# vrgamegirl19/comfyui-vrgamedevgirl

Measured on AMD Instinct MI355X. Metric: Mpixels/s (grain+LUT+colormatch+sharpen) at 4K, higher is better.
Workload: dtype f32

## Files before the change

comfyui-vrgamedevgirl_amd/csrc/vrg_chain.hip:

```cpp
#include "vrg_common.hpp"
#include <type_traits>
#include "vrg_chain_stages.hpp"

namespace vrg {

constexpr int STATS_BPF_MAX = 128;
constexpr int STATS_PX_PER_BLOCK = 16384;

__host__ __device__ inline int stats_blocks_per_frame(int64_t pixels) {
    int64_t b = (pixels + STATS_PX_PER_BLOCK - 1) / STATS_PX_PER_BLOCK;
    return (int)(b < 1 ? 1 : (b > STATS_BPF_MAX ? STATS_BPF_MAX : b));
}

template <int STAGES, class IO>
__global__ __launch_bounds__(256) void k_chain_pointwise(const typename IO::elem* __restrict__ in, typename IO::elem* __restrict__ out,
                                                          int32_t ppf, ChainK D) {
    VRG_CM_MATH(PT, (STAGES & VRG_STAGE_COLORMATCH) != 0, (STAGES & VRG_STAGE_FASTMATH) != 0, D.dm);
    const int32_t p = blockIdx.x * 256 + threadIdx.x;
    if (p >= ppf) return;
    const int64_t f = blockIdx.y;
    const px3 v = IO::load_stream(in + f * ppf + p);
    const float x[3] = {v.r, v.g, v.b};
    float o[3];
    chain_pre<STAGES>(D, frame_ctx<STAGES>(D, f), p, x, o, PT);
// ... 8 lines not shown
    px3 v[4];
#pragma unroll
    for (int j = 0; j < 4; ++j) {
        const int32_t p = p0 + 256 * j;
        v[j] = load_px_stream(fin + (p < ppf ? p : 0));
    }
    VRG_CM_MATH(PT, true, (STAGES & VRG_STAGE_FASTMATH) != 0, D.dm);
    typedef unsigned u3 __attribute__((ext_vector_type(3)));
    const __amdgpu_buffer_rsrc_t rs = __builtin_amdgcn_make_buffer_rsrc(reinterpret_cast<void*>(out + f * ppf), 0, ppf * 12, 0x00020000);
    const FrameCtx FC = frame_ctx<STAGES>(D, f);
#pragma unroll
    for (int j = 0; j < 4; ++j) {
        const int32_t p = p0 + 256 * j;
        const bool valid = p < ppf;
        const float x[3] = {v[j].r, v[j].g, v[j].b};
        float o[3];
        chain_pre<STAGES>(D, FC, valid ? p : 0, x, o, PT);
        __builtin_amdgcn_raw_buffer_store_b96(u3{__float_as_uint(o[0]), __float_as_uint(o[1]), __float_as_uint(o[2])}, rs,
                                              (int)(valid ? (uint32_t)p * 12u : 0x80000000u), 0, 0);
    }
}

#define VRG_TILE_H 32
constexpr int TILE_H = VRG_TILE_H, TILE_W = 64;
constexpr int TILE_ROWS = TILE_H / 4;
constexpr int HALO_H = TILE_H + 2, HALO_W = TILE_W + 2;
constexpr int LDS_PITCH = HALO_W + 1;

template <int STAGES, class IO>
__global__ __launch_bounds__(256) void k_chain_tile(const typename IO::elem* __restrict__ in, typename IO::elem* __restrict__ out,
                                                     int32_t H, int32_t W, int32_t tiles_x, int32_t tiles_per_frame, uint32_t total_work,
                                                     ChainK D) {
    __shared__ float tile[3][HALO_H][LDS_PITCH];
    VRG_CM_MATH(PT, (STAGES & VRG_STAGE_COLORMATCH) != 0, (STAGES & VRG_STAGE_FASTMATH) != 0, D.dm);
    const uint32_t per_xcd = (total_work + 7u) / 8u;
    const uint32_t work = (blockIdx.x & 7u) * per_xcd + (blockIdx.x >> 3);
    if ((blockIdx.x >> 3) >= per_xcd || work >= total_work) return;
    const uint32_t tile_id = work % (uint32_t)tiles_per_frame;
    const int32_t ty0 = (int32_t)(tile_id / (uint32_t)tiles_x) * TILE_H;
    const int32_t tx0 = (int32_t)(tile_id % (uint32_t)tiles_x) * TILE_W;
    const int64_t f = work / (uint32_t)tiles_per_frame;
    const int32_t ppf = H * W;
    const typename IO::elem* fin = in + f * ppf;
    const bool zero = D.zero_border != 0;
    const FrameCtx FC = frame_ctx<STAGES>(D, f);

#define VRG_TILE_PRELOAD 1
    constexpr int N_IT = (HALO_H * HALO_W + 255) / 256;
    if (VRG_TILE_PRELOAD && !(STAGES & VRG_STAGE_COLORMATCH) && !((STAGES & VRG_STAGE_GRAIN) && !(STAGES & VRG_STAGE_LUT))) {
        px3 v[N_IT];
        int32_t pp[N_IT];
#pragma unroll
        for (int k = 0; k < N_IT; ++k) {
            int i = (int)threadIdx.x + 256 * k;
            i = i < HALO_H * HALO_W ? i : 0;
            const int hy = i / HALO_W, hx = i - hy * HALO_W;
            int y = ty0 + hy - 1, x = tx0 + hx - 1;
            y = y < 0 ? 0 : (y > H - 1 ? H - 1 : y);
            x = x < 0 ? 0 : (x > W - 1 ? W - 1 : x);
            pp[k] = y * W + x;
            v[k] = IO::load(fin + pp[k]);
        }
#pragma unroll
        for (int k = 0; k < N_IT; ++k) {
            const int i = (int)threadIdx.x + 256 * k;
            if (i < HALO_H * HALO_W) {
                const int hy = i / HALO_W, hx = i - hy * HALO_W;
// ... 448 lines not shown
```

comfyui-vrgamedevgirl_amd/csrc/vrg_common.hpp:

```cpp
#pragma once

#if !defined(VRG_LAB_VARIANT_SOURCE) && (defined(VRG_APPLY_EARLY_LOAD) || defined(VRG_APPLY_ROWS) || defined(VRG_FLAT_ROWS) || defined(VRG_GRAIN_NT) || \
    defined(VRG_PRODUCE_MAX_WAVES_LABONLY) || defined(VRG_PRODUCE_WAVES) || defined(VRG_PRODUCE_WAVES_LABONLY) || defined(VRG_PR_PIPE) || \
    defined(VRG_PR_SUBS) || defined(VRG_SG_PIPE) || defined(VRG_TILE_H) || defined(VRG_TILE_PRELOAD) || \
    defined(VRG_TS_LANES) || defined(VRG_TS_LANES_DEPTH) || defined(VRG_TS_LANES_MAX_FRAMES) || defined(VRG_TS_LANES_MEAN_DEPTH) || \
    defined(VRG_TS_MARKSTEIN) || defined(VRG_TS_ROWS_DEPTH) || defined(VRG_TS_ROWS_MAX_FRAMES) || defined(VRG_TS_SPLIT_DEPTH) || \
    defined(VRG_TS_SPLIT_MAX_FRAMES) || defined(VRG_TS_WHOLE_DEPTH) || defined(VRG_ZIV_REL) || defined(VRG_MARCH_FAST) || \
    defined(VRG_MARCH_MIN_WAVES) || defined(VRG_MARCH_FINITE) || defined(VRG_MARCH_ABLATE) || defined(VRG_MARCH_QUAD) || \
    defined(VRG_MARCH_ENDIO) || defined(VRG_MARCH_ROTATE) || defined(VRG_MARCH_TAPS_UNFOLD) || defined(VRG_MARCH_FAST_FLAT) || \
    defined(VRG_MARCH_EDGE_SHARED) || defined(VRG_MARCH_FAST_LDS) || defined(VRG_NO_POINTWISE4) || defined(VRG_NO_APPLY_MARCH) || \
    defined(VRG_NO_FLAT_STENCIL) || defined(VRG_APPLY_FORCE_GENERAL) || defined(VRG_ABLATE_GATHER) || defined(VRG_NO_DIVT_FASTPATH))
#error "comfyui-vrgamedevgirl_amd: tuning / ablation macros are not build options of the product sources (see the note above this line)"
#endif
#include <stdint.h>

#include "../../include/vrgdg_hip.h"
#include "../../include/vrgdg_hip_debug.h"
#include "vrg_pixel_math.hpp"

namespace vrg {

VRG_HD bool span_fits(int64_t offset, int64_t need, int64_t size) { return offset >= 0 && offset <= size && need <= size - offset; }

constexpr int64_t LAUNCH_RECORDS = 32768;
// ... 72 lines not shown
    int64_t chunk0;
    int64_t frame_elems;
    int32_t chunk_frames;
    uint32_t G;
};

VRG_HD uint64_t chunk_seed(const NoiseK& n, int64_t chunk_rel) { return n.seed0 + (uint64_t)(n.chunk0 + chunk_rel) * n.seed_stride; }
VRG_HD uint64_t chunk_offset(const NoiseK& n, int64_t chunk_rel) { return n.off0 + (uint64_t)(n.chunk0 + chunk_rel) * n.off_stride; }

struct CmK {
    const float* img_ms;
    const float* ref_ms;
    int32_t ref_frames;
    float K, T;
};

struct ChainK {
    int32_t stages;
    float I, S, T;
    NoiseK noise;
    LutParams lut;
    CmK cm;
    DevMath dm;
    int32_t stencil_op, zero_border;
    float strength;
};

constexpr int VRG_STAGE_FASTMATH = 32;

inline DevMath host_dev_math() { return DevMath{(float)2.4, (float)(1.0 / 2.4), (float)(1.0 / 3.0), nullptr}; }

template <bool FAST> struct CmMathSel { typedef DevMath type; };
template <> struct CmMathSel<true> { typedef PowTables type; };
__device__ __forceinline__ PowTables cm_make_math(const float* lds, const DevMath&, const PowTables*) { return PowTables{lds, lds + 512}; }
__device__ __forceinline__ DevMath cm_make_math(const float* lds, const DevMath& dm, const DevMath*) {
    DevMath m = dm;
    m.logt = lds;
    return m;
}

inline NoiseK make_noise(const vrg_noise_desc* d, int64_t frame_elems) {
    NoiseK n;
    n.seed0 = d->seed0; n.seed_stride = d->seed_stride; n.off0 = d->offset0; n.off_stride = d->offset_stride;
    n.chunk0 = d->chunk0; n.frame_elems = frame_elems; n.chunk_frames = d->chunk_frames; n.G = d->grid_threads;
    return n;
}

inline LutParams make_lut(const float* cells, int n, const float dmin[3], const float dmax[3], int blend_mode,
                          float blend, float one_minus_blend) {
    LutParams P;
    P.cells = cells; P.n = n; P.top = (float)(n - 1);
    P.unit_domain = 1;
    for (int c = 0; c < 3; ++c) {
        P.dmin[c] = dmin[c];
        const float span = dmax[c] - dmin[c];
        P.span[c] = span < 1e-6f ? 1e-6f : span;
        if (!(P.dmin[c] == 0.0f && P.span[c] == 1.0f)) P.unit_domain = 0;
    }
    P.blend_mode = blend_mode; P.blend = blend; P.one_minus_blend = one_minus_blend;
    return P;
}

#define VRG_CM_MATH(PT, NEED, FAST, DM)                                                                       \
    __shared__ __attribute__((aligned(16))) float vrg_pow_lds_[(NEED) ? ((FAST) ? ::vrg::POW_TABLE_WORDS : ::vrg::ZIV_TABLE_WORDS) : 4]; \
    if (NEED) {                                                                                                \
        if (FAST) ::vrg::pow_tables_fill(vrg_pow_lds_, (int)threadIdx.x, (int)blockDim.x);                    \
        else ::vrg::ziv_table_fill(vrg_pow_lds_, (int)threadIdx.x, (int)blockDim.x);                          \
        __syncthreads();                                                                                       \
    }                                                                                                          \
    typedef typename ::vrg::CmMathSel<(FAST)>::type PT##_t;                                                    \
    const PT##_t PT = ::vrg::cm_make_math(vrg_pow_lds_, (DM), (const PT##_t*)nullptr)

#define VRG_CHECK_LAUNCH()                                   \
    do {                                                     \
        hipError_t e_ = hipGetLastError();                   \
        if (e_ != hipSuccess) return VRG_ERR_LAUNCH;         \
    } while (0)

template <class T, int N>
__device__ __forceinline__ void block_sum_4waves(T (&acc)[N], T (&part)[4][N]) {
#pragma unroll
    for (int i = 0; i < N; ++i) {
#pragma unroll
        for (int off = 32; off >= 1; off >>= 1) acc[i] += __shfl_xor(acc[i], off, 64);
    }
    const int wave = threadIdx.x >> 6, lane = threadIdx.x & 63;
    if (lane == 0) {
#pragma unroll
        for (int i = 0; i < N; ++i) part[wave][i] = acc[i];
    }
    __syncthreads();
}

}
#endif
```

comfyui-vrgamedevgirl_amd/csrc/vrg_pixel_math.hpp:

```cpp
#pragma once
#include <stdint.h>

#if defined(__HIPCC__) || defined(__HIP__)
#include <hip/hip_runtime.h>
#define VRG_HD __host__ __device__ __forceinline__
#define VRG_D __device__ __forceinline__
#else
#define VRG_HD inline
#define VRG_D inline
#endif

#ifndef VRG_HW_LOG2
#define VRG_HW_LOG2(x) __builtin_amdgcn_logf(x)
#define VRG_HW_SIN_REV(x) __builtin_amdgcn_sinf(x)
#define VRG_HW_COS_REV(x) __builtin_amdgcn_cosf(x)
#define VRG_HW_EXP2(x) __builtin_amdgcn_exp2f(x)
#define VRG_HW_RCP(x) __builtin_amdgcn_rcpf(x)
#endif

namespace vrg {

VRG_HD float f32_from_bits(uint32_t b) {
    union { uint32_t u; float f; } c;
    c.u = b;
// ... 428 lines not shown
VRG_HD void pow_tables_fill(float* dst, int first, int stride) {
    for (int i = first; i < POW_TABLE_WORDS; i += stride)
        dst[i] = f32_from_bits(i < 512 ? VRG_POW_LOGT[i >> 2][i & 3] : VRG_POW_EXPT[(i - 512) >> 1][(i - 512) & 1]);
}

VRG_HD float pow_pos(float x, float y, const PowTables& T) {
    union { float f; uint32_t u; } cv;
    cv.f = x;
    const uint32_t b = cv.u;
    const float e = (float)((int)(b >> 23) - 127);
    const uint32_t i = (b >> 16) & 0x7fu;
    const float m = f32_from_bits((b & 0x007fffffu) | 0x3f800000u);
    const float invc = T.logt[4 * i], lhi = T.logt[4 * i + 1], llo = T.logt[4 * i + 2];
    const float r = __builtin_fmaf(m, invc, -1.0f);
    float p = __builtin_fmaf(r, f32_from_bits(VRG_POW_A[2]), f32_from_bits(VRG_POW_A[1]));
    p = __builtin_fmaf(r, p, f32_from_bits(VRG_POW_A[0]));
    const float L_hi = e + lhi;
    const float L_lo = __builtin_fmaf(r, p, llo);
    const float E_hi = y * L_hi;
    const float E_lo = __builtin_fmaf(y, L_lo, __builtin_fmaf(y, L_hi, -E_hi));
    const float nf = __builtin_rintf(E_hi * 64.0f);
    const float f = __builtin_fmaf(nf, -0.015625f, E_hi) + E_lo;
    const int n = (int)nf;
    float q = __builtin_fmaf(f, f32_from_bits(VRG_POW_B[3]), f32_from_bits(VRG_POW_B[2]));
    q = __builtin_fmaf(f, q, f32_from_bits(VRG_POW_B[1]));
    q = __builtin_fmaf(f, q, f32_from_bits(VRG_POW_B[0]));
    q = f * q;
    const float thi = T.expt[2 * (n & 63)], tlo = T.expt[2 * (n & 63) + 1];
    const float v = thi + __builtin_fmaf(thi, q, tlo);
    const float res = __builtin_ldexpf(v, n >> 6);
    return (x != x) ? x : res;
}

struct DevMath {
    float e24, e1_24, e1_3;
    const float* logt;
};

#if defined(__HIP_DEVICE_COMPILE__)
extern "C" __device__ float __ocml_pow_f32(float, float);
#define VRG_LIB_POWF(x, y) __ocml_pow_f32((x), (y))
#define VRG_HW_FREXP_MANT(x) __builtin_amdgcn_frexp_mantf(x)
#define VRG_HW_FREXP_EXP(x) __builtin_amdgcn_frexp_expf(x)
#else
#define VRG_LIB_POWF(x, y) __builtin_powf((x), (y))
#define VRG_HW_FREXP_MANT(x) __builtin_frexpf((x), &vrg_frexp_dummy_)
#define VRG_HW_FREXP_EXP(x) ::vrg::host_frexp_exp(x)
static int vrg_frexp_dummy_;
VRG_HD int host_frexp_exp(float x) { int e; (void)__builtin_frexpf(x, &e); return e; }
#endif

constexpr int DEV_POW_ANY = 0, DEV_POW_OVF = 1, DEV_POW_UNIT = 2;

VRG_HD float dev_exp_core(float x) {
    const float c = f32_from_bits(0x3fb8aa3bu);
    const float ph = x * c;
    const float f0 = __builtin_fmaf(x, c, -ph);
    const float pl = __builtin_fmaf(x, f32_from_bits(0x32a5705fu), f0);
    const float e = __builtin_rintf(ph);
    const float a = (ph - e) + pl;
    return __builtin_ldexpf(VRG_HW_EXP2(a), (int)e);
}

VRG_HD float dev_exp_core_normal(float x) {
    const float c = f32_from_bits(0x3fb8aa3bu);
    const float ph = x * c;
    const float f0 = __builtin_fmaf(x, c, -ph);
    const float pl = __builtin_fmaf(x, f32_from_bits(0x32a5705fu), f0);
    const float magic = f32_from_bits(0x4b400000u);
// ... 119 lines not shown
    float ln_hi, ln_lo;
    dev_epln<GUARD>(x, ln_hi, ln_lo);
    const float p17 = y * ln_hi;
    const float p24 = __builtin_fmaf(y, ln_hi, -p17);
    const float p44 = __builtin_fmaf(y, ln_lo, p24);
    const float p50 = p17 + p44;
    const float p51 = p50 - p17;
    const float p52 = p44 - p51;
    const float inf = __builtin_inff();
    const float ovf = f32_from_bits(0x42b17218u);
    float ph = p50, pl = p52;
    if (GUARD == DEV_POW_ANY) {
        ph = (__builtin_fabsf(p17) == inf) ? p17 : p50;
        pl = (__builtin_fabsf(ph) == inf) ? 0.0f : p52;
    }
    float h5 = ph, l7 = pl;
    if (GUARD != DEV_POW_UNIT) {
        const float c4 = (ph == ovf) ? f32_from_bits(0x37000000u) : 0.0f;
        h5 = ph - c4;
        l7 = pl + c4;
    }
    float e8 = dev_exp_core(h5);
    if (GUARD == DEV_POW_ANY) e8 = (h5 < f32_from_bits(0xc2ce8ed0u)) ? 0.0f : e8;
    if (GUARD != DEV_POW_UNIT) e8 = (h5 > ovf) ? inf : e8;
    const float r9 = __builtin_fmaf(e8, l7, e8);
    const float r = (GUARD != DEV_POW_UNIT && __builtin_fabsf(e8) == inf) ? e8 : r9;
    if (GUARD == DEV_POW_ANY) return (x == inf) ? (y > 0.0f ? inf : 0.0f) : r;
    return (x < inf) ? r : ((x == inf) ? (y > 0.0f ? inf : 0.0f) : x);
}
VRG_HD float dev_pow(float x, float y) { return dev_pow_t<DEV_POW_ANY>(x, y); }

#include "vrg_ziv_log_table.inc"

constexpr int ZIV_TABLE_WORDS = 128 * 4;

VRG_HD void ziv_table_fill(float* dst, int first, int stride) {
    for (int i = first; i < ZIV_TABLE_WORDS; i += stride) dst[i] = f32_from_bits(VRG_ZIV_LOGT[i >> 2][i & 3]);
}

VRG_HD void ziv_log(float x, const float* T, float& Lh, float& Ll, float& Eh_out, float& A_out) {
    const int32_t d = (int32_t)(f32_bits(x) - 0x3f2aaaabu);
    const uint32_t e23 = (uint32_t)d & 0xff800000u;
    const float ef23 = (float)(int32_t)e23;
    const float m = f32_from_bits(f32_bits(x) - e23);
    const float* t = T + (((uint32_t)d >> 16) & 0x7fu) * 4;
    const float c = t[0], th = t[1], tl = t[2];
    A_out = t[3];
    const float r = __builtin_fmaf(m, c, -1.0f);
    const float Eh = ef23 * f32_from_bits(0x33b17200u);
    const float h = r * r;
    const float l = __builtin_fmaf(r, r, -h);
    float P = __builtin_fmaf(r, (float)(-1.0 / 6.0), 0.2f);
    P = __builtin_fmaf(r, P, -0.25f);
    P = __builtin_fmaf(r, P, (float)(1.0 / 3.0));
    const float tail = __builtin_fmaf(-0.5f, l, (h * r) * P);
    const float s1 = Eh + th;
    const float s2 = __builtin_fmaf(-0.5f, h, r);
    const float e2 = __builtin_fmaf(-0.5f, h, r - s2);
    const float s3 = s1 + s2;
    const float e3 = s2 - (s3 - s1);
    float low = __builtin_fmaf(ef23, f32_from_bits(0x2a3fbe8eu), tl);
    low = low + e3;
    low = low + e2;
    low = low + tail;
    Lh = s3;
    Ll = low;
    Eh_out = Eh;
}

#define VRG_ZIV_REL 1
#define VRG_ZIV_REL_BITS 0x2e06f428u
VRG_HD float ziv_delta(float Lh, float Eh, float A_over_C) {
#if VRG_ZIV_REL
    const float rel = __builtin_fmaf(__builtin_fabsf(Eh), 64.0f, __builtin_fabsf(Lh));
#if defined(__HIP_DEVICE_COMPILE__)
    return __builtin_amdgcn_fmed3f(rel, A_over_C, 0.0f);
#else
    return __builtin_fminf(rel, A_over_C);
#endif
#else
    (void)Lh; (void)Eh;
    return A_over_C;
#endif
}

template <bool IN_DOMAIN = false>
VRG_HD bool ziv_try(float x, float y, const float* T, uint32_t lo_bits, uint32_t hi_bits, float& out) {
    float Lh, Ll, Eh, A;
    ziv_log(x, T, Lh, Ll, Eh, A);
    const float p17 = y * Lh;
    const float p24 = __builtin_fmaf(y, Lh, -p17);
    const float p44 = __builtin_fmaf(y, Ll, p24);
    const float yc = y * f32_from_bits(VRG_ZIV_REL_BITS);
    const float dl = ziv_delta(Lh, Eh, A);
    const float up = __builtin_fmaf(yc, dl, p44), dn = __builtin_fmaf(-yc, dl, p44);
    const float php = p17 + up;
    const float phm = p17 + dn;
    const float t = php - p17;
    const float e8 = dev_exp_core_normal(php);
    const float rp = __builtin_fmaf(e8, up - t, e8);
    const float rm = __builtin_fmaf(e8, dn - t, e8);
    out = rp;
    if (IN_DOMAIN) return (php == phm) & (rp == rm);
    return ((f32_bits(x) - lo_bits) <= (hi_bits - lo_bits)) & (php == phm) & (rp == rm);
}

template <int GUARD>
VRG_HD float dev_pow_ziv(float x, float y, const float* T, uint32_t lo_bits, uint32_t hi_bits) {
#if defined(__HIP_DEVICE_COMPILE__)
    if (T) {
        float r;
        if (ziv_try(x, y, T, lo_bits, hi_bits, r)) return r;
#if defined(VRG_LAB_VARIANT_SOURCE) && defined(LAB_ZIV_NO_FALLBACK)
        return r;
#endif
    }
#else
    (void)T; (void)lo_bits; (void)hi_bits;
#endif
    return dev_pow_t<GUARD>(x, y);
}

template <int GUARD, bool IN_DOMAIN = false>
VRG_HD void dev_pow_ziv3(const float x[3], float y, const float* T, uint32_t lo_bits, uint32_t hi_bits, float o[3]) {
#if defined(__HIP_DEVICE_COMPILE__)
    if (T) {
        float r0, r1, r2;
        const bool dom = IN_DOMAIN || __builtin_fmaxf(__builtin_fmaxf(x[0], x[1]), x[2]) <= f32_from_bits(hi_bits);
        const bool s0 = ziv_try<true>(x[0], y, T, lo_bits, hi_bits, r0) & dom;
        const bool s1 = ziv_try<true>(x[1], y, T, lo_bits, hi_bits, r1) & dom;
        const bool s2 = ziv_try<true>(x[2], y, T, lo_bits, hi_bits, r2) & dom;
        o[0] = r0; o[1] = r1; o[2] = r2;
#if defined(VRG_LAB_VARIANT_SOURCE) && defined(LAB_ZIV_NO_FALLBACK)
        if (s0 | s1 | s2 | true) return;
#endif
        if (!s0) o[0] = dev_pow_t<GUARD>(x[0], y);
        if (!s1) o[1] = dev_pow_t<GUARD>(x[1], y);
        if (!s2) o[2] = dev_pow_t<GUARD>(x[2], y);
        return;
    }
#else
    (void)T; (void)lo_bits; (void)hi_bits;
#endif
#pragma unroll
    for (int c = 0; c < 3; ++c) o[c] = dev_pow_t<GUARD>(x[c], y);
}

VRG_HD float cm_div_scalar(float x, float c, float rc, float, const PowTables&) { return div_const(x, c, rc); }
VRG_HD float cm_div_scalar(float x, float, float, float rc_dev, const DevMath&) { return x * rc_dev; }
#define VRG_CM_DIVS(x, c, M) ::vrg::cm_div_scalar((x), (float)(c), 1.0f / (float)(c), (float)(1.0 / (double)(c)), (M))
VRG_HD float cm_div_tensor(float x, float c, float rc, const PowTables&) { return div_const(x, c, rc); }
VRG_HD float cm_div_tensor(float x, float c, float rc, const DevMath&) {
#if defined(__HIP_DEVICE_COMPILE__)
    const bool proven = ((__builtin_fabsf(x) - 1e-30f) <= (1e30f - 1e-30f)) | (x == 0.0f);
    if (__builtin_amdgcn_ballot_w64(!proven) == 0) return div_const(x, c, rc);
#else
    (void)rc;
#endif
    return x / c;
// ... 281 lines not shown
```

comfyui-vrgamedevgirl_amd/csrc/vrg_probe.hip:

```cpp
#include "vrg_common.hpp"
#include "vrg_lanes.hpp"
#include "vrg_tstats_config.hpp"

namespace vrg {

__global__ __launch_bounds__(256) void k_selftest_divconst(unsigned long long* counts, uint32_t first) {
    const uint32_t bits = first + blockIdx.x * 256u + threadIdx.x;
    const float x = f32_from_bits(bits);
    if (x != x) return;
    const float a = __builtin_fabsf(x);
    const bool mid = a >= 1e-30f && a <= 1e30f;
    float got[9], want[9];
    got[0] = VRG_DIVC(x, 1.055f);   want[0] = x / 1.055f;
    got[1] = VRG_DIVC(x, 12.92f);   want[1] = x / 12.92f;
    got[2] = VRG_DIVC(x, 0.95047f); want[2] = x / 0.95047f;
    got[3] = VRG_DIVC(x, 1.08883f); want[3] = x / 1.08883f;
    got[4] = VRG_DIVC(x, 116.0f);   want[4] = x / 116.0f;
    got[5] = VRG_DIVC(x, 500.0f);   want[5] = x / 500.0f;
    got[6] = VRG_DIVC(x, 200.0f);   want[6] = x / 200.0f;
    got[7] = VRG_DIVC(x, 7.787f);   want[7] = x / 7.787f;
    got[8] = div9(x);               want[8] = x / 9.0f;
#pragma unroll
    for (int w = 0; w < 9; ++w) {
        const bool same = (got[w] == want[w]) || (got[w] != got[w] && want[w] != want[w]);
// ... 180 lines not shown
            acc[j] = 0.0f;
        }
        for (int pass = 0; pass < 3; ++pass) {
            __syncthreads();
            const f32x4* src = reinterpret_cast<const f32x4*>(cells + (size_t)pass * total);
            f32x4* dst = reinterpret_cast<f32x4*>(dbg_nodes);
            for (int i = threadIdx.x; i < (total + 3) / 4; i += 1024) dst[i] = src[i];
            __syncthreads();
            const float* T = dbg_nodes;
#pragma unroll
            for (int j = 0; j < PX; ++j) {
                const int bs = base[j];
                acc[j] += (T[bs] + T[bs + 1]) + (T[bs + n] + T[bs + n + 1]);
                acc[j] += (T[bs + n * n] + T[bs + n * n + 1]) + (T[bs + n * n + n] + T[bs + n * n + n + 1]);
            }
        }
#pragma unroll
        for (int j = 0; j < PX; ++j) {
            const int64_t p = b0 + j * 1024 + threadIdx.x;
            if (p < pixels) out[p] = acc[j];
        }
    }
}

__global__ __launch_bounds__(256) void k_dbg_cm_math(const float* __restrict__ in, float* __restrict__ out, int64_t n, int op, float y,
                                                      DevMath dm) {
    VRG_CM_MATH(PT, true, true, dm);
    __shared__ __attribute__((aligned(16))) float zivt[ZIV_TABLE_WORDS];
    ziv_table_fill(zivt, (int)threadIdx.x, 256);
    __syncthreads();
    dm.logt = zivt;
    const int64_t i = (int64_t)blockIdx.x * 256 + threadIdx.x;
    if (i >= n) return;
    if (op == 20) {
        const float lab = in[3 * i], mu = in[3 * i + 1], sd = in[3 * i + 2];
        const float ms[6] = {mu, sd, mu, sd, mu, sd};
        const SigmaRecip R = sigma_recip(ms);
        const float d = lab - mu;
        out[3 * i] = div_sigma_unscaled(d, sd, R.y1[0]);
        out[3 * i + 1] = d / sd;
        out[3 * i + 2] = (R.usable && (__builtin_fabsf(d) + __builtin_fabsf(d)) + __builtin_fabsf(d) < 0x1p40f) ? 1.0f : 0.0f;
    } else if (op >= 16) {
        float a, b;
        float eh, aj;
        if (op <= 17) dev_epln<DEV_POW_UNIT>(in[i], a, b); else ziv_log(in[i], zivt, a, b, eh, aj);
        out[i] = (op & 1) ? b : a;
    } else if (op >= 12) {
        const float x = in[i];
        if (op == 12) out[i] = dev_pow_ziv<DEV_POW_OVF>(x, y, zivt, 0x3d800000u, 0x40000000u);
        else if (op == 13) out[i] = dev_pow_ziv<DEV_POW_UNIT>(x, y, zivt, 0x3b4d2e1cu, 0x40800000u);
        else if (op == 14) out[i] = dev_pow_ziv<DEV_POW_UNIT>(x, y, zivt, 0x3c1118c2u, 0x40800000u);
        else {
            float r;
            out[i] = ziv_try(x, y, zivt, 0x00800000u, 0x7f7fffffu, r) ? 0.0f : 1.0f;
        }
    } else if (op >= 9) {
        out[i] = op == 9 ? dev_pow_t<DEV_POW_ANY>(in[i], y) : (op == 10 ? dev_pow_t<DEV_POW_OVF>(in[i], y) : dev_pow_t<DEV_POW_UNIT>(in[i], y));
    } else if (op <= 4) {
        const float x = in[i];
        float r;
        if (op == 0) r = VRG_LIB_POWF(x, y);
        else if (op == 1) r = x * (float)(1.0 / (double)y);
        else if (op == 2) r = x / y;
        else if (op == 3) r = pow_pos(x, y, PT);
        else r = cbrt_pow(x);
        out[i] = r;
    } else {
        const float x[3] = {in[3 * i], in[3 * i + 1], in[3 * i + 2]};
        float o[3];
        if (op == 5) rgb_to_lab(x, o, dm);
        else if (op == 6) lab_to_rgb(x, o, dm);
        else if (op == 7) rgb_to_lab(x, o, PT);
        else lab_to_rgb(x, o, PT);
        out[3 * i] = o[0]; out[3 * i + 1] = o[1]; out[3 * i + 2] = o[2];
    }
}

}

namespace vrg {

template <int MODE>
__global__ __launch_bounds__(256) void k_dbg_copy(const f32x4* __restrict__ in, f32x4* __restrict__ out, int64_t n4) {
    if (MODE == 0 || MODE == 1) {
        const int64_t i = (int64_t)blockIdx.x * 256 + threadIdx.x;
        if (i >= n4) return;
        if (MODE == 0) out[i] = in[i];
// ... 308 lines not shown
    hipStream_t st = (hipStream_t)stream;
#define VRG_VALU_CASE(M) case M: hipLaunchKernelGGL(vrg::k_dbg_valu_rate<M>, dim3(blocks), dim3(256), 0, st, out, iters); break;
    switch (mode) {
        VRG_VALU_CASE(0) VRG_VALU_CASE(1) VRG_VALU_CASE(2) VRG_VALU_CASE(3) VRG_VALU_CASE(4) VRG_VALU_CASE(5) VRG_VALU_CASE(6) VRG_VALU_CASE(7) VRG_VALU_CASE(8) VRG_VALU_CASE(9) VRG_VALU_CASE(10) VRG_VALU_CASE(11) VRG_VALU_CASE(12) VRG_VALU_CASE(13) VRG_VALU_CASE(14) VRG_VALU_CASE(15) VRG_VALU_CASE(16) VRG_VALU_CASE(17) VRG_VALU_CASE(18) VRG_VALU_CASE(19) VRG_VALU_CASE(20) VRG_VALU_CASE(21) VRG_VALU_CASE(30) VRG_VALU_CASE(31) VRG_VALU_CASE(32) VRG_VALU_CASE(33) VRG_VALU_CASE(34) VRG_VALU_CASE(35) VRG_VALU_CASE(36) VRG_VALU_CASE(37) VRG_VALU_CASE(38) VRG_VALU_CASE(39) VRG_VALU_CASE(40) VRG_VALU_CASE(41) VRG_VALU_CASE(42) VRG_VALU_CASE(43) VRG_VALU_CASE(44) VRG_VALU_CASE(45) VRG_VALU_CASE(46) VRG_VALU_CASE(47) VRG_VALU_CASE(48) VRG_VALU_CASE(49) VRG_VALU_CASE(50) VRG_VALU_CASE(51) VRG_VALU_CASE(52) VRG_VALU_CASE(53) VRG_VALU_CASE(54) VRG_VALU_CASE(55) VRG_VALU_CASE(56) VRG_VALU_CASE(57) VRG_VALU_CASE(60) VRG_VALU_CASE(61) VRG_VALU_CASE(62) VRG_VALU_CASE(63) VRG_VALU_CASE(64) VRG_VALU_CASE(65) VRG_VALU_CASE(66) VRG_VALU_CASE(67) VRG_VALU_CASE(68) VRG_VALU_CASE(69) VRG_VALU_CASE(72) VRG_VALU_CASE(73)
        default: return VRG_ERR_BAD_ARG;
    }
#undef VRG_VALU_CASE
    VRG_CHECK_LAUNCH();
    return VRG_OK;
}

int vrg_debug_copy_f32(const float* in, float* out, int64_t n_floats, int32_t mode, void* stream) {
    if (!in || !out || n_floats <= 0 || (n_floats & 3) || mode < 0 || mode > 4) return VRG_ERR_BAD_ARG;
    if ((reinterpret_cast<uintptr_t>(in) | reinterpret_cast<uintptr_t>(out)) & 15) return VRG_ERR_BAD_ARG;
    const int64_t n4 = n_floats / 4;
    const int64_t per_block = (mode == 2 || mode == 3) ? 1024 : 256;
    const uint64_t blocks = (uint64_t)((n4 + per_block - 1) / per_block);
    if (blocks > 0x7fffffffull) return VRG_ERR_UNSUPPORTED;
    const vrg::f32x4* src = reinterpret_cast<const vrg::f32x4*>(in);
    vrg::f32x4* dst = reinterpret_cast<vrg::f32x4*>(out);
    hipStream_t st = (hipStream_t)stream;
    switch (mode) {
        case 0: hipLaunchKernelGGL(vrg::k_dbg_copy<0>, dim3((uint32_t)blocks), dim3(256), 0, st, src, dst, n4); break;
        case 1: hipLaunchKernelGGL(vrg::k_dbg_copy<1>, dim3((uint32_t)blocks), dim3(256), 0, st, src, dst, n4); break;
        case 2: hipLaunchKernelGGL(vrg::k_dbg_copy<2>, dim3((uint32_t)blocks), dim3(256), 0, st, src, dst, n4); break;
        case 3: hipLaunchKernelGGL(vrg::k_dbg_copy<3>, dim3((uint32_t)blocks), dim3(256), 0, st, src, dst, n4); break;
        default: hipLaunchKernelGGL(vrg::k_dbg_copy<4>, dim3((uint32_t)blocks), dim3(256), 0, st, src, dst, n4); break;
    }
    VRG_CHECK_LAUNCH();
    return VRG_OK;
}

int vrg_debug_cm_math(const float* in, float* out, int64_t n, int32_t op, float y, void* stream) {
    if (!in || !out || n <= 0 || op < 0 || op > 20) return VRG_ERR_BAD_ARG;
    const uint64_t blocks = (uint64_t)(n + 255) / 256;
    if (blocks > 0x7fffffffull) return VRG_ERR_UNSUPPORTED;
    hipLaunchKernelGGL(vrg::k_dbg_cm_math, dim3((uint32_t)blocks), dim3(256), 0, (hipStream_t)stream, in, out, n, op, y, vrg::host_dev_math());
    VRG_CHECK_LAUNCH();
    return VRG_OK;
}

int vrg_debug_lut_fetch(const float* in, float* out, int64_t pixels, const float* cells, int32_t lut_size, int32_t mode, void* stream) {
    if (!in || !out || !cells || pixels <= 0 || lut_size < 2 || mode < 0 || mode > 19) return VRG_ERR_BAD_ARG;
    const uint32_t blocks = (uint32_t)((pixels + 255) / 256);
    const vrg::px3* src = reinterpret_cast<const vrg::px3*>(in);
    if (mode >= 9) {
        switch (mode) {
            case 9: hipLaunchKernelGGL(vrg::k_dbg_lut_fetch_r4<9>, dim3(blocks), dim3(256), 0, (hipStream_t)stream, src, out, pixels, cells, lut_size); break;
            case 10: hipLaunchKernelGGL(vrg::k_dbg_lut_fetch_r4<10>, dim3(blocks), dim3(256), 0, (hipStream_t)stream, src, out, pixels, cells, lut_size); break;
            case 11: hipLaunchKernelGGL(vrg::k_dbg_lut_fetch_r4<11>, dim3(blocks), dim3(256), 0, (hipStream_t)stream, src, out, pixels, cells, lut_size); break;
            case 12: hipLaunchKernelGGL(vrg::k_dbg_lut_fetch_r4<12>, dim3(blocks), dim3(256), 0, (hipStream_t)stream, src, out, pixels, cells, lut_size); break;
            case 13: hipLaunchKernelGGL(vrg::k_dbg_lut_fetch_r4<13>, dim3(blocks), dim3(256), 0, (hipStream_t)stream, src, out, pixels, cells, lut_size); break;
            case 14: hipLaunchKernelGGL(vrg::k_dbg_lut_fetch_r4<14>, dim3(blocks), dim3(256), 0, (hipStream_t)stream, src, out, pixels, cells, lut_size); break;
            case 15: hipLaunchKernelGGL(vrg::k_dbg_lut_fetch_r4<15>, dim3(blocks), dim3(256), 0, (hipStream_t)stream, src, out, pixels, cells, lut_size); break;
            case 16: hipLaunchKernelGGL(vrg::k_dbg_lut_fetch_r4<16>, dim3(blocks), dim3(256), 0, (hipStream_t)stream, src, out, pixels, cells, lut_size); break;
            case 17: hipLaunchKernelGGL(vrg::k_dbg_lut_fetch_r4<17>, dim3(blocks), dim3(256), 0, (hipStream_t)stream, src, out, pixels, cells, lut_size); break;
            case 18: hipLaunchKernelGGL(vrg::k_dbg_lut_fetch_r4<18>, dim3(blocks), dim3(256), 0, (hipStream_t)stream, src, out, pixels, cells, lut_size); break;
            default: hipLaunchKernelGGL(vrg::k_dbg_lut_fetch_r4<19>, dim3(blocks), dim3(256), 0, (hipStream_t)stream, src, out, pixels, cells, lut_size); break;
        }
        VRG_CHECK_LAUNCH();
        return VRG_OK;
    }
    if (mode >= 7) {
        const size_t lds = ((size_t)lut_size * lut_size * lut_size * 4 + 15) / 16 * 16;
        if (lds > 160 * 1024) return VRG_ERR_UNSUPPORTED;
        int dev = 0, cus = 256;
        if (hipGetDevice(&dev) != hipSuccess || hipDeviceGetAttribute(&cus, hipDeviceAttributeMultiprocessorCount, dev) != hipSuccess) cus = 256;
// ... 53 lines not shown
```

comfyui-vrgamedevgirl_amd/csrc/vrg_produce.hip:

```cpp
#include "vrg_produce_body.hpp"

namespace vrg {

#define VRG_PRODUCE_MAX_WAVES_LABONLY 8
template <int STAGES, bool TWO_PART, bool STATS = true>
__global__ __launch_bounds__(256, TWO_PART ? 1 : (STATS ? VRG_PRODUCE_WAVES : VRG_PRODUCE_WAVES_LABONLY)) void k_produce_lab(const float* __restrict__ in, float* __restrict__ lab_out, ProduceK P, ChainK D,
                                                      const float* __restrict__ pivots, double* __restrict__ rec,
                                                      int32_t* __restrict__ rec_frame) {
    constexpr int CAP = (!TWO_PART && !STATS) ? VRG_PRODUCE_MAX_WAVES_LABONLY : 8;
    constexpr int PAD = CAP >= 8 ? 16 : (160 * 1024 / (CAP + 1) + 512 - 14400 > 16 ? 160 * 1024 / (CAP + 1) + 512 - 14400 : 16);
    __shared__ char occupancy_pad[PAD];
    if (P.numel < 0) occupancy_pad[threadIdx.x] = (char)blockIdx.x;
    __shared__ float sn[4][PR_SUB + 4];
    __shared__ double red[STATS ? 4 : 1][12];
    VRG_CM_MATH(PT, true, (STAGES & VRG_STAGE_FASTMATH) != 0, D.dm);
    produce_lab_body<STAGES, TWO_PART, STATS>(blockIdx.x, in, lab_out, P, D, pivots, rec, rec_frame, sn, red, PT);
}

template <int STAGES>
__global__ __launch_bounds__(64) void k_frame_pivots(const px3* __restrict__ in, int32_t ppf, int64_t frames, ChainK D, float* __restrict__ pivots) {
    VRG_CM_MATH(PT, true, (STAGES & VRG_STAGE_FASTMATH) != 0, D.dm);
    const int64_t f = (int64_t)blockIdx.x * 64 + threadIdx.x;
    if (f >= frames) return;
    const px3 v0 = in[f * ppf];
    const float x0[3] = {v0.r, v0.g, v0.b};
    float pre[3], lab[3];
    chain_pre<STAGES>(D, frame_ctx<STAGES>(D, f), 0, x0, pre, PT);
    rgb_to_lab(pre, lab, PT);
    pivots[f * 3] = lab[0]; pivots[f * 3 + 1] = lab[1]; pivots[f * 3 + 2] = lab[2];
}

__global__ __launch_bounds__(256) void k_produce_merge(const double* __restrict__ rec, const int32_t* __restrict__ rec_frame,
                                                        const float* __restrict__ pivots, uint32_t recs_per_chunk, int32_t chunk_frames,
                                                        int32_t ppf, double* __restrict__ stats) {
    __shared__ double red[4][6];
    const int32_t f = blockIdx.x;
    const int64_t first = (int64_t)(f / chunk_frames) * recs_per_chunk;
    double acc[6] = {0.0, 0.0, 0.0, 0.0, 0.0, 0.0};
    for (uint32_t r = threadIdx.x; r < recs_per_chunk; r += 256) {
        if (rec_frame[first + r] == f) {
#pragma unroll
            for (int i = 0; i < 6; ++i) acc[i] += rec[(first + r) * 6 + i];
        }
    }
    const int lane = threadIdx.x & 63, wave = threadIdx.x >> 6;
#pragma unroll
    for (int i = 0; i < 6; ++i) {
        const double a = wave_sum_f64(acc[i]);
// ... 68 lines not shown
```

Measured before the change: 42040.

## Use per-binade Ziv log table to drop exponent split in pow

Adds an 11-binade log table in which each entry folds in the exponent terms, so the Ziv log path indexes by raw float bits and skips the exponent extraction, the extra FMAs and the relative-error computation per call. Kernels that can afford it (produce with stats) get the larger LDS table. The tile kernel and the lab-only produce kernel keep the old 128-entry table to save LDS and fill time. The cost is a bigger LDS footprint and a longer table fill where the large table is used.

```diff
diff --git a/comfyui-vrgamedevgirl_amd/csrc/vrg_chain.hip b/comfyui-vrgamedevgirl_amd/csrc/vrg_chain.hip
--- a/comfyui-vrgamedevgirl_amd/csrc/vrg_chain.hip
+++ b/comfyui-vrgamedevgirl_amd/csrc/vrg_chain.hip
@@ -64,7 +64,7 @@
                                                      int32_t H, int32_t W, int32_t tiles_x, int32_t tiles_per_frame, uint32_t total_work,
                                                      ChainK D) {
     __shared__ float tile[3][HALO_H][LDS_PITCH];
-    VRG_CM_MATH(PT, (STAGES & VRG_STAGE_COLORMATCH) != 0, (STAGES & VRG_STAGE_FASTMATH) != 0, D.dm);
+    VRG_CM_MATH_128(PT, (STAGES & VRG_STAGE_COLORMATCH) != 0, (STAGES & VRG_STAGE_FASTMATH) != 0, D.dm);
     const uint32_t per_xcd = (total_work + 7u) / 8u;
     const uint32_t work = (blockIdx.x & 7u) * per_xcd + (blockIdx.x >> 3);
     if ((blockIdx.x >> 3) >= per_xcd || work >= total_work) return;
diff --git a/comfyui-vrgamedevgirl_amd/csrc/vrg_common.hpp b/comfyui-vrgamedevgirl_amd/csrc/vrg_common.hpp
--- a/comfyui-vrgamedevgirl_amd/csrc/vrg_common.hpp
+++ b/comfyui-vrgamedevgirl_amd/csrc/vrg_common.hpp
@@ -128,10 +128,10 @@
 
 template <bool FAST> struct CmMathSel { typedef DevMath type; };
 template <> struct CmMathSel<true> { typedef PowTables type; };
-__device__ __forceinline__ PowTables cm_make_math(const float* lds, const DevMath&, const PowTables*) { return PowTables{lds, lds + 512}; }
-__device__ __forceinline__ DevMath cm_make_math(const float* lds, const DevMath& dm, const DevMath*) {
+__device__ __forceinline__ PowTables cm_make_math(const float* lds, int, const DevMath&, const PowTables*) { return PowTables{lds, lds + 512}; }
+__device__ __forceinline__ DevMath cm_make_math(const float* lds, int binades, const DevMath& dm, const DevMath*) {
     DevMath m = dm;
-    m.logt = lds;
+    m.logt = ZivT(lds, binades);
     return m;
 }
 
@@ -157,15 +157,18 @@
     return P;
 }
 
-#define VRG_CM_MATH(PT, NEED, FAST, DM)                                                                       \
-    __shared__ __attribute__((aligned(16))) float vrg_pow_lds_[(NEED) ? ((FAST) ? ::vrg::POW_TABLE_WORDS : ::vrg::ZIV_TABLE_WORDS) : 4]; \
+#define VRG_CM_MATH_Z(PT, NEED, FAST, DM, BINADES)                                                            \
+    __shared__ __attribute__((aligned(16))) float vrg_pow_lds_[(NEED) ? ((FAST) ? ::vrg::POW_TABLE_WORDS : ((BINADES) ? ::vrg::ZIV_TABLE_WORDS : ::vrg::ZIV_TABLE128_WORDS)) : 4]; \
     if (NEED) {                                                                                                \
         if (FAST) ::vrg::pow_tables_fill(vrg_pow_lds_, (int)threadIdx.x, (int)blockDim.x);                    \
-        else ::vrg::ziv_table_fill(vrg_pow_lds_, (int)threadIdx.x, (int)blockDim.x);                          \
+        else if (BINADES) ::vrg::ziv_table_fill(vrg_pow_lds_, (int)threadIdx.x, (int)blockDim.x);             \
+        else ::vrg::ziv_table_fill128(vrg_pow_lds_, (int)threadIdx.x, (int)blockDim.x);                       \
         __syncthreads();                                                                                       \
     }                                                                                                          \
     typedef typename ::vrg::CmMathSel<(FAST)>::type PT##_t;                                                    \
-    const PT##_t PT = ::vrg::cm_make_math(vrg_pow_lds_, (DM), (const PT##_t*)nullptr)
+    const PT##_t PT = ::vrg::cm_make_math(vrg_pow_lds_, (BINADES), (DM), (const PT##_t*)nullptr)
+#define VRG_CM_MATH(PT, NEED, FAST, DM) VRG_CM_MATH_Z(PT, NEED, FAST, DM, ::vrg::ZIV_BINADES)
+#define VRG_CM_MATH_128(PT, NEED, FAST, DM) VRG_CM_MATH_Z(PT, NEED, FAST, DM, 0)
 
 #define VRG_CHECK_LAUNCH()                                   \
     do {                                                     \
diff --git a/comfyui-vrgamedevgirl_amd/csrc/vrg_pixel_math.hpp b/comfyui-vrgamedevgirl_amd/csrc/vrg_pixel_math.hpp
--- a/comfyui-vrgamedevgirl_amd/csrc/vrg_pixel_math.hpp
+++ b/comfyui-vrgamedevgirl_amd/csrc/vrg_pixel_math.hpp
@@ -484,9 +484,16 @@
     return (x != x) ? x : res;
 }
 
+constexpr int ZIV_E_MIN = -8;
+constexpr int ZIV_BINADES = 11;
+struct ZivT {
+    const float* p;
+    int binades;
+    VRG_HD constexpr ZivT(const float* q = nullptr, int b = ZIV_BINADES) : p(q), binades(b) {}
+};
 struct DevMath {
     float e24, e1_24, e1_3;
-    const float* logt;
+    ZivT logt;
 };
 
 #if defined(__HIP_DEVICE_COMPILE__)
@@ -672,45 +679,70 @@
 
 #include "vrg_ziv_log_table.inc"
 
-constexpr int ZIV_TABLE_WORDS = 128 * 4;
+constexpr int ZIV_ENTRIES = ZIV_BINADES * 128;
+constexpr int ZIV_TABLE_WORDS = ZIV_ENTRIES * 4;
+constexpr uint32_t ZIV_INDEX_BASE = 0x3f2aaaabu - ((uint32_t)(-ZIV_E_MIN) << 23);
+
+VRG_HD void ziv_table_entry(int i, float w[4]) {
+    const int e = (i >> 7) + ZIV_E_MIN, j = i & 127;
+    const float ef23 = (float)(e * (1 << 23));
+    w[0] = f32_from_bits(VRG_ZIV_LOGT[j][0] - ((uint32_t)e << 23));
+    w[1] = ef23 * f32_from_bits(0x33b17200u) + f32_from_bits(VRG_ZIV_LOGT[j][1]);
+    w[2] = __builtin_fmaf(ef23, f32_from_bits(0x2a3fbe8eu), f32_from_bits(VRG_ZIV_LOGT[j][2]));
+    w[3] = f32_from_bits(VRG_ZIV_LOGT[j][3] | (e != 0 ? 0x80000000u : 0u));
+}
 
 VRG_HD void ziv_table_fill(float* dst, int first, int stride) {
-    for (int i = first; i < ZIV_TABLE_WORDS; i += stride) dst[i] = f32_from_bits(VRG_ZIV_LOGT[i >> 2][i & 3]);
-}
-
-VRG_HD void ziv_log(float x, const float* T, float& Lh, float& Ll, float& Eh_out, float& A_out) {
-    const int32_t d = (int32_t)(f32_bits(x) - 0x3f2aaaabu);
-    const uint32_t e23 = (uint32_t)d & 0xff800000u;
-    const float ef23 = (float)(int32_t)e23;
-    const float m = f32_from_bits(f32_bits(x) - e23);
-    const float* t = T + (((uint32_t)d >> 16) & 0x7fu) * 4;
-    const float c = t[0], th = t[1], tl = t[2];
-    A_out = t[3];
-    const float r = __builtin_fmaf(m, c, -1.0f);
-    const float Eh = ef23 * f32_from_bits(0x33b17200u);
+    for (int i = first; i < ZIV_ENTRIES; i += stride) {
+        float w[4];
+        ziv_table_entry(i, w);
+        dst[4 * i] = w[0]; dst[4 * i + 1] = w[1]; dst[4 * i + 2] = w[2]; dst[4 * i + 3] = w[3];
+    }
+}
+
+constexpr int ZIV_TABLE128_WORDS = 128 * 4;
+VRG_HD void ziv_table_fill128(float* dst, int first, int stride) {
+    for (int i = first; i < ZIV_TABLE128_WORDS; i += stride) dst[i] = f32_from_bits(VRG_ZIV_LOGT[i >> 2][i & 3]);
+}
+
+VRG_HD uint32_t ziv_index(float x) {
+    const uint32_t i = (f32_bits(x) - ZIV_INDEX_BASE) >> 16;
+    return i < (uint32_t)(ZIV_ENTRIES - 1) ? i : (uint32_t)(ZIV_ENTRIES - 1);
+}
+
+VRG_HD void ziv_log_sum(float r, float s1, float tl, float& Lh, float& Ll) {
     const float h = r * r;
     const float l = __builtin_fmaf(r, r, -h);
     float P = __builtin_fmaf(r, (float)(-1.0 / 6.0), 0.2f);
     P = __builtin_fmaf(r, P, -0.25f);
     P = __builtin_fmaf(r, P, (float)(1.0 / 3.0));
     const float tail = __builtin_fmaf(-0.5f, l, (h * r) * P);
-    const float s1 = Eh + th;
     const float s2 = __builtin_fmaf(-0.5f, h, r);
     const float e2 = __builtin_fmaf(-0.5f, h, r - s2);
     const float s3 = s1 + s2;
     const float e3 = s2 - (s3 - s1);
-    float low = __builtin_fmaf(ef23, f32_from_bits(0x2a3fbe8eu), tl);
-    low = low + e3;
+    float low = tl + e3;
     low = low + e2;
     low = low + tail;
     Lh = s3;
     Ll = low;
-    Eh_out = Eh;
 }
 
 #define VRG_ZIV_REL 1
 #define VRG_ZIV_REL_BITS 0x2e06f428u
-VRG_HD float ziv_delta(float Lh, float Eh, float A_over_C) {
+VRG_HD float ziv_delta(float Lh, float W) {
+#if VRG_ZIV_REL
+#if defined(__HIP_DEVICE_COMPILE__)
+    return __builtin_fabsf(__builtin_amdgcn_fmed3f(__builtin_fabsf(Lh), W, -1.0f));
+#else
+    return __builtin_fabsf(__builtin_fminf(__builtin_fabsf(Lh), W));
+#endif
+#else
+    (void)Lh;
+    return __builtin_fabsf(W);
+#endif
+}
+VRG_HD float ziv_delta128(float Lh, float Eh, float A_over_C) {
 #if VRG_ZIV_REL
     const float rel = __builtin_fmaf(__builtin_fabsf(Eh), 64.0f, __builtin_fabsf(Lh));
 #if defined(__HIP_DEVICE_COMPILE__)
@@ -724,15 +756,36 @@
 #endif
 }
 
+VRG_HD void ziv_log(float x, const ZivT T, float& Lh, float& Ll, float& dl) {
+    if (T.binades) {
+        const float* t = T.p + ziv_index(x) * 4;
+        const float c = t[0], s1 = t[1], tl = t[2], W = t[3];
+        const float r = __builtin_fmaf(x, c, -1.0f);
+        ziv_log_sum(r, s1, tl, Lh, Ll);
+        dl = ziv_delta(Lh, W);
+        return;
+    }
+    const int32_t d = (int32_t)(f32_bits(x) - 0x3f2aaaabu);
+    const uint32_t e23 = (uint32_t)d & 0xff800000u;
+    const float ef23 = (float)(int32_t)e23;
+    const float m = f32_from_bits(f32_bits(x) - e23);
+    const float* t = T.p + (((uint32_t)d >> 16) & 0x7fu) * 4;
+    const float c = t[0], th = t[1], tl = t[2], A = t[3];
+    const float r = __builtin_fmaf(m, c, -1.0f);
+    const float Eh = ef23 * f32_from_bits(0x33b17200u);
+    const float s1 = Eh + th;
+    ziv_log_sum(r, s1, __builtin_fmaf(ef23, f32_from_bits(0x2a3fbe8eu), tl), Lh, Ll);
+    dl = ziv_delta128(Lh, Eh, A);
+}
+
 template <bool IN_DOMAIN = false>
-VRG_HD bool ziv_try(float x, float y, const float* T, uint32_t lo_bits, uint32_t hi_bits, float& out) {
-    float Lh, Ll, Eh, A;
-    ziv_log(x, T, Lh, Ll, Eh, A);
+VRG_HD bool ziv_try(float x, float y, const ZivT T, uint32_t lo_bits, uint32_t hi_bits, float& out) {
+    float Lh, Ll, dl;
+    ziv_log(x, T, Lh, Ll, dl);
     const float p17 = y * Lh;
     const float p24 = __builtin_fmaf(y, Lh, -p17);
     const float p44 = __builtin_fmaf(y, Ll, p24);
     const float yc = y * f32_from_bits(VRG_ZIV_REL_BITS);
-    const float dl = ziv_delta(Lh, Eh, A);
     const float up = __builtin_fmaf(yc, dl, p44), dn = __builtin_fmaf(-yc, dl, p44);
     const float php = p17 + up;
     const float phm = p17 + dn;
@@ -746,9 +799,9 @@
 }
 
 template <int GUARD>
-VRG_HD float dev_pow_ziv(float x, float y, const float* T, uint32_t lo_bits, uint32_t hi_bits) {
-#if defined(__HIP_DEVICE_COMPILE__)
-    if (T) {
+VRG_HD float dev_pow_ziv(float x, float y, const ZivT T, uint32_t lo_bits, uint32_t hi_bits) {
+#if defined(__HIP_DEVICE_COMPILE__)
+    if (T.p) {
         float r;
         if (ziv_try(x, y, T, lo_bits, hi_bits, r)) return r;
 #if defined(VRG_LAB_VARIANT_SOURCE) && defined(LAB_ZIV_NO_FALLBACK)
@@ -762,9 +815,9 @@
 }
 
 template <int GUARD, bool IN_DOMAIN = false>
-VRG_HD void dev_pow_ziv3(const float x[3], float y, const float* T, uint32_t lo_bits, uint32_t hi_bits, float o[3]) {
-#if defined(__HIP_DEVICE_COMPILE__)
-    if (T) {
+VRG_HD void dev_pow_ziv3(const float x[3], float y, const ZivT T, uint32_t lo_bits, uint32_t hi_bits, float o[3]) {
+#if defined(__HIP_DEVICE_COMPILE__)
+    if (T.p) {
         float r0, r1, r2;
         const bool dom = IN_DOMAIN || __builtin_fmaxf(__builtin_fmaxf(x[0], x[1]), x[2]) <= f32_from_bits(hi_bits);
         const bool s0 = ziv_try<true>(x[0], y, T, lo_bits, hi_bits, r0) & dom;
diff --git a/comfyui-vrgamedevgirl_amd/csrc/vrg_probe.hip b/comfyui-vrgamedevgirl_amd/csrc/vrg_probe.hip
--- a/comfyui-vrgamedevgirl_amd/csrc/vrg_probe.hip
+++ b/comfyui-vrgamedevgirl_amd/csrc/vrg_probe.hip
@@ -236,7 +236,9 @@
     dm.logt = zivt;
     const int64_t i = (int64_t)blockIdx.x * 256 + threadIdx.x;
     if (i >= n) return;
-    if (op == 20) {
+    if (op == 21) {
+        out[i] = zivt[i % ZIV_TABLE_WORDS];
+    } else if (op == 20) {
         const float lab = in[3 * i], mu = in[3 * i + 1], sd = in[3 * i + 2];
         const float ms[6] = {mu, sd, mu, sd, mu, sd};
         const SigmaRecip R = sigma_recip(ms);
@@ -246,8 +248,8 @@
         out[3 * i + 2] = (R.usable && (__builtin_fabsf(d) + __builtin_fabsf(d)) + __builtin_fabsf(d) < 0x1p40f) ? 1.0f : 0.0f;
     } else if (op >= 16) {
         float a, b;
-        float eh, aj;
-        if (op <= 17) dev_epln<DEV_POW_UNIT>(in[i], a, b); else ziv_log(in[i], zivt, a, b, eh, aj);
+        float aj;
+        if (op <= 17) dev_epln<DEV_POW_UNIT>(in[i], a, b); else ziv_log(in[i], zivt, a, b, aj);
         out[i] = (op & 1) ? b : a;
     } else if (op >= 12) {
         const float x = in[i];
@@ -256,7 +258,7 @@
         else if (op == 14) out[i] = dev_pow_ziv<DEV_POW_UNIT>(x, y, zivt, 0x3c1118c2u, 0x40800000u);
         else {
             float r;
-            out[i] = ziv_try(x, y, zivt, 0x00800000u, 0x7f7fffffu, r) ? 0.0f : 1.0f;
+            out[i] = ziv_try(x, y, zivt, 0x3b4d2e1cu, 0x40800000u, r) ? 0.0f : 1.0f;
         }
     } else if (op >= 9) {
         out[i] = op == 9 ? dev_pow_t<DEV_POW_ANY>(in[i], y) : (op == 10 ? dev_pow_t<DEV_POW_OVF>(in[i], y) : dev_pow_t<DEV_POW_UNIT>(in[i], y));
@@ -631,7 +633,7 @@
 }
 
 int vrg_debug_cm_math(const float* in, float* out, int64_t n, int32_t op, float y, void* stream) {
-    if (!in || !out || n <= 0 || op < 0 || op > 20) return VRG_ERR_BAD_ARG;
+    if (!in || !out || n <= 0 || op < 0 || op > 21) return VRG_ERR_BAD_ARG;
     const uint64_t blocks = (uint64_t)(n + 255) / 256;
     if (blocks > 0x7fffffffull) return VRG_ERR_UNSUPPORTED;
     hipLaunchKernelGGL(vrg::k_dbg_cm_math, dim3((uint32_t)blocks), dim3(256), 0, (hipStream_t)stream, in, out, n, op, y, vrg::host_dev_math());
diff --git a/comfyui-vrgamedevgirl_amd/csrc/vrg_produce.hip b/comfyui-vrgamedevgirl_amd/csrc/vrg_produce.hip
--- a/comfyui-vrgamedevgirl_amd/csrc/vrg_produce.hip
+++ b/comfyui-vrgamedevgirl_amd/csrc/vrg_produce.hip
@@ -2,6 +2,7 @@
 
 namespace vrg {
 
+#define VRG_PRODUCE_LABONLY_BINADES 0
 #define VRG_PRODUCE_MAX_WAVES_LABONLY 8
 template <int STAGES, bool TWO_PART, bool STATS = true>
 __global__ __launch_bounds__(256, TWO_PART ? 1 : (STATS ? VRG_PRODUCE_WAVES : VRG_PRODUCE_WAVES_LABONLY)) void k_produce_lab(const float* __restrict__ in, float* __restrict__ lab_out, ProduceK P, ChainK D,
@@ -13,7 +14,7 @@
     if (P.numel < 0) occupancy_pad[threadIdx.x] = (char)blockIdx.x;
     __shared__ float sn[4][PR_SUB + 4];
     __shared__ double red[STATS ? 4 : 1][12];
-    VRG_CM_MATH(PT, true, (STAGES & VRG_STAGE_FASTMATH) != 0, D.dm);
+    VRG_CM_MATH_Z(PT, true, (STAGES & VRG_STAGE_FASTMATH) != 0, D.dm, (!TWO_PART && !STATS) ? VRG_PRODUCE_LABONLY_BINADES : ::vrg::ZIV_BINADES);
     produce_lab_body<STAGES, TWO_PART, STATS>(blockIdx.x, in, lab_out, P, D, pivots, rec, rec_frame, sn, red, PT);
 }
 
```

Result: no change. 42390, median of 6 (+0.8%).
